# SEAME-pt/Team02-ObjectDetection

Hardware: NVIDIA B200
Metric: MobileNetV2UNet inference images/s (higher is better)
Workload: dtype bf16

## Files before the change

team02-objectdetection_b200/csrc/common.cuh:

```cuda
#pragma once
#include <cuda_runtime.h>
#include <cuda_bf16.h>
#include <cuda.h>
#include <stdint.h>
#include <stdio.h>

#include "../../include/b200seg.h"

namespace b200 {

int set_error(int code, const char* fmt, ...);
int check_launch(const char* what);
int sm_count();

int pdl_mode();
template <typename... KA, typename... A>
inline cudaError_t launch_pdl_if(bool on, void (*kern)(KA...), dim3 grid, dim3 block, size_t smem, cudaStream_t st, A... args) {
  cudaLaunchConfig_t cfg = {};
  cfg.gridDim = grid;
  cfg.blockDim = block;
  cfg.dynamicSmemBytes = smem;
  cfg.stream = st;
  cudaLaunchAttribute at[1];
  at[0].id = cudaLaunchAttributeProgrammaticStreamSerialization;
  at[0].val.programmaticStreamSerializationAllowed = 1;
  cfg.attrs = at;
  cfg.numAttrs = on ? 1 : 0;
  return cudaLaunchKernelEx(&cfg, kern, KA(args)...);
}
template <typename... KA, typename... A>
inline cudaError_t launch_pdl(void (*kern)(KA...), dim3 grid, dim3 block, size_t smem, cudaStream_t st, A... args) {
  const int m = pdl_mode();
  return launch_pdl_if(m == 1 || m == 3, kern, grid, block, smem, st, args...);
}

#define B200_REQUIRE(cond, ...)                                   \
  do {                                                            \
    if (!(cond)) return ::b200::set_error(-1, __VA_ARGS__);       \
  } while (0)

int make_tmap_bf16(CUtensorMap* out, const void* base, int rank, const uint64_t* dims,
                   const uint64_t* strides_bytes, const uint32_t* box, int swizzle128,
                   const uint32_t* elem_strides = nullptr);

#ifdef __CUDACC__

__device__ __forceinline__ uint32_t smem_u32(const void* p) {
  return static_cast<uint32_t>(__cvta_generic_to_shared(p));
}
__device__ __forceinline__ uint64_t globaltimer_ns() {
  uint64_t t;
  asm volatile("mov.u64 %0, %%globaltimer;" : "=l"(t));
  return t;
}

__device__ __forceinline__ void mbar_init(uint64_t* bar, uint32_t count) {
  asm volatile("mbarrier.init.shared::cta.b64 [%0], %1;" ::"r"(smem_u32(bar)), "r"(count) : "memory");
}
__device__ __forceinline__ void fence_barrier_init() {
  asm volatile("fence.mbarrier_init.release.cluster;" ::: "memory");
}
__device__ __forceinline__ void mbar_arrive_expect_tx(uint64_t* bar, uint32_t bytes) {
  asm volatile("mbarrier.arrive.expect_tx.shared::cta.b64 _, [%0], %1;" ::"r"(smem_u32(bar)), "r"(bytes)
               : "memory");
}
__device__ __forceinline__ void mbar_arrive(uint64_t* bar) {
  asm volatile("mbarrier.arrive.shared::cta.b64 _, [%0];" ::"r"(smem_u32(bar)) : "memory");
}
__device__ __forceinline__ bool mbar_try_wait(uint64_t* bar, uint32_t parity) {
  uint32_t ok;
  asm volatile(
      "{\n\t.reg .pred p;\n\t"
      "mbarrier.try_wait.parity.shared::cta.b64 p, [%1], %2;\n\t"
      "selp.u32 %0, 1, 0, p;\n\t}"
      : "=r"(ok)
      : "r"(smem_u32(bar)), "r"(parity)
      : "memory");
  return ok != 0;
}
__device__ __forceinline__ void mbar_wait(uint64_t* bar, uint32_t parity, int tag = 0) {
  if (mbar_try_wait(bar, parity)) return;
  const uint64_t t0 = globaltimer_ns();
  uint32_t spins = 0;
  while (!mbar_try_wait(bar, parity)) {
    if ((++spins & 0x3ff) == 0 && globaltimer_ns() - t0 > 2000000000ull) {
      printf("b200seg: mbarrier wait timeout tag=%d block=(%d,%d) thread=%d parity=%u\n", tag, blockIdx.x,
             blockIdx.y, threadIdx.x, parity);
      __trap();
    }
  }
}

__device__ __forceinline__ void pdl_wait() { asm volatile("griddepcontrol.wait;" ::: "memory"); }
__device__ __forceinline__ void pdl_trigger() { asm volatile("griddepcontrol.launch_dependents;" ::: "memory"); }

__device__ __forceinline__ bool elect_one() {
  uint32_t pred;
  asm volatile(
      "{\n\t.reg .pred P;\n\t"
      "elect.sync _|P, 0xffffffff;\n\t"
      "selp.u32 %0, 1, 0, P;\n\t}"
      : "=r"(pred));
  return pred != 0;
}

__device__ __forceinline__ void fence_proxy_async_smem() {
  asm volatile("fence.proxy.async.shared::cta;" ::: "memory");
}
__device__ __forceinline__ void tc_fence_before() { asm volatile("tcgen05.fence::before_thread_sync;" ::: "memory"); }
__device__ __forceinline__ void tc_fence_after() { asm volatile("tcgen05.fence::after_thread_sync;" ::: "memory"); }
__device__ __forceinline__ void named_bar_sync(int id, int nthreads) {
  asm volatile("bar.sync %0, %1;" ::"r"(id), "r"(nthreads) : "memory");
}

__device__ __forceinline__ void tma_prefetch_desc(const CUtensorMap* m) {
  asm volatile("prefetch.tensormap [%0];" ::"l"(m) : "memory");
}
__device__ __forceinline__ void tma_load_3d(void* dst, const CUtensorMap* m, uint64_t* bar, int c0, int c1,
                                            int c2) {
  asm volatile(
      "cp.async.bulk.tensor.3d.shared::cluster.global.mbarrier::complete_tx::bytes [%0], [%1, {%3, %4, %5}], [%2];"
      ::"r"(smem_u32(dst)), "l"(m), "r"(smem_u32(bar)), "r"(c0), "r"(c1), "r"(c2)
      : "memory");
}
__device__ __forceinline__ void tma_load_4d(void* dst, const CUtensorMap* m, uint64_t* bar, int c0, int c1,
                                            int c2, int c3) {
  asm volatile(
      "cp.async.bulk.tensor.4d.shared::cluster.global.mbarrier::complete_tx::bytes [%0], [%1, {%3, %4, %5, %6}], [%2];"
      ::"r"(smem_u32(dst)), "l"(m), "r"(smem_u32(bar)), "r"(c0), "r"(c1), "r"(c2), "r"(c3)
      : "memory");
}
__device__ __forceinline__ void tma_store_4d(const CUtensorMap* m, const void* src, int c0, int c1, int c2,
                                             int c3) {
  asm volatile("cp.async.bulk.tensor.4d.global.shared::cta.bulk_group [%0, {%2, %3, %4, %5}], [%1];" ::"l"(m),
               "r"(smem_u32(src)), "r"(c0), "r"(c1), "r"(c2), "r"(c3)
               : "memory");
}
__device__ __forceinline__ void tma_store_commit() { asm volatile("cp.async.bulk.commit_group;" ::: "memory"); }
__device__ __forceinline__ void tma_store_wait_all() { asm volatile("cp.async.bulk.wait_group 0;" ::: "memory"); }

__device__ __forceinline__ void tmem_alloc(uint32_t* dst_smem, uint32_t ncols) {
  asm volatile("tcgen05.alloc.cta_group::1.sync.aligned.shared::cta.b32 [%0], %1;" ::"r"(smem_u32(dst_smem)),
               "r"(ncols)
               : "memory");
}
__device__ __forceinline__ void tmem_relinquish() {
  asm volatile("tcgen05.relinquish_alloc_permit.cta_group::1.sync.aligned;" ::: "memory");
}
__device__ __forceinline__ void tmem_dealloc(uint32_t taddr, uint32_t ncols) {
  asm volatile("tcgen05.dealloc.cta_group::1.sync.aligned.b32 %0, %1;" ::"r"(taddr), "r"(ncols) : "memory");
}
__device__ __forceinline__ void umma_bf16(uint32_t d_tmem, uint64_t a_desc, uint64_t b_desc, uint32_t idesc,
                                          uint32_t accumulate) {
  asm volatile(
      "{\n\t.reg .pred p;\n\t"
      "setp.ne.b32 p, %4, 0;\n\t"
      "tcgen05.mma.cta_group::1.kind::f16 [%0], %1, %2, %3, p;\n\t}"
      ::"r"(d_tmem), "l"(a_desc), "l"(b_desc), "r"(idesc), "r"(accumulate)
      : "memory");
}
__device__ __forceinline__ void umma_bf16_lohi(uint32_t d_tmem, uint32_t a_lo, uint32_t b_lo, uint32_t desc_hi,
                                               uint32_t idesc, uint32_t accumulate) {
  asm volatile(
      "{\n\t.reg .pred p;\n\t.reg .b64 da, db;\n\t"
      "setp.ne.b32 p, %5, 0;\n\t"
      "mov.b64 da, {%1, %3};\n\t"
      "mov.b64 db, {%2, %3};\n\t"
      "tcgen05.mma.cta_group::1.kind::f16 [%0], da, db, %4, p;\n\t}"
      ::"r"(d_tmem), "r"(a_lo), "r"(b_lo), "r"(desc_hi), "r"(idesc), "r"(accumulate)
      : "memory");
}
__device__ __forceinline__ void umma_commit(uint64_t* bar) {
  asm volatile("tcgen05.commit.cta_group::1.mbarrier::arrive::one.shared::cluster.b64 [%0];" ::"r"(smem_u32(bar))
               : "memory");
}
__device__ __forceinline__ void tmem_ld16(uint32_t taddr, uint32_t (&r)[16]) {
  asm volatile(
      "tcgen05.ld.sync.aligned.32x32b.x16.b32 {%0, %1, %2, %3, %4, %5, %6, %7, %8, %9, %10, %11, %12, %13, %14, %15}, [%16];"
      : "=r"(r[0]), "=r"(r[1]), "=r"(r[2]), "=r"(r[3]), "=r"(r[4]), "=r"(r[5]), "=r"(r[6]), "=r"(r[7]),
        "=r"(r[8]), "=r"(r[9]), "=r"(r[10]), "=r"(r[11]), "=r"(r[12]), "=r"(r[13]), "=r"(r[14]), "=r"(r[15])
      : "r"(taddr)
      : "memory");
}
__device__ __forceinline__ void tmem_ld8(uint32_t taddr, uint32_t (&r)[16]) {
  asm volatile("tcgen05.ld.sync.aligned.32x32b.x8.b32 {%0, %1, %2, %3, %4, %5, %6, %7}, [%8];"
               : "=r"(r[0]), "=r"(r[1]), "=r"(r[2]), "=r"(r[3]), "=r"(r[4]), "=r"(r[5]), "=r"(r[6]), "=r"(r[7])
               : "r"(taddr)
               : "memory");
}
__device__ __forceinline__ void tmem_ld_wait() { asm volatile("tcgen05.wait::ld.sync.aligned;" ::: "memory"); }

__device__ __forceinline__ uint64_t umma_desc_k128(uint32_t smem_addr) {
  uint64_t d = 0;
  d |= (uint64_t)((smem_addr & 0x3FFFF) >> 4);
  d |= (uint64_t)1 << 16;
  d |= (uint64_t)(1024 >> 4) << 32;
  d |= (uint64_t)1 << 46;
  d |= (uint64_t)2 << 61;
  return d;
}
__device__ __forceinline__ uint64_t umma_desc_nosw(uint32_t smem_addr, uint32_t lbo_bytes, uint32_t sbo_bytes) {
  uint64_t d = 0;
  d |= (uint64_t)((smem_addr & 0x3FFFF) >> 4);
  d |= (uint64_t)(lbo_bytes >> 4) << 16;
  d |= (uint64_t)(sbo_bytes >> 4) << 32;
  d |= (uint64_t)1 << 46;
  return d;
}
__host__ __device__ __forceinline__ uint32_t umma_idesc_bf16(int M, int N) {
  return (1u << 4) | (1u << 7) | (1u << 10) | ((uint32_t)(N >> 3) << 17) | ((uint32_t)(M >> 4) << 24);
}

template <int ACT>
__device__ __forceinline__ float apply_act(float v) {
  if (ACT == B200SEG_ACT_RELU) return fmaxf(v, 0.f);
  if (ACT == B200SEG_ACT_RELU6) return fminf(fmaxf(v, 0.f), 6.f);
  return v;
}
__device__ __forceinline__ float apply_act_rt(float v, int act) {
  if (act == B200SEG_ACT_RELU) return fmaxf(v, 0.f);
  if (act == B200SEG_ACT_RELU6) return fminf(fmaxf(v, 0.f), 6.f);
  return v;
}
__device__ __forceinline__ uint32_t pack_bf16x2(float lo, float hi) {
  __nv_bfloat162 h = __floats2bfloat162_rn(lo, hi);
  return *reinterpret_cast<uint32_t*>(&h);
}
__device__ __forceinline__ float bf16lo(uint32_t u) { return __uint_as_float(u << 16); }
__device__ __forceinline__ float bf16hi(uint32_t u) { return __uint_as_float(u & 0xffff0000u); }

__device__ __forceinline__ float fma_bf16_lo(uint32_t a, uint32_t b, float c) {
  float d;
  asm("{.reg .b16 al, ah, bl, bh; mov.b32 {al, ah}, %1; mov.b32 {bl, bh}, %2; fma.rn.f32.bf16 %0, al, bl, %3;}"
      : "=f"(d) : "r"(a), "r"(b), "f"(c));
  return d;
}
__device__ __forceinline__ float fma_bf16_hi(uint32_t a, uint32_t b, float c) {
  float d;
  asm("{.reg .b16 al, ah, bl, bh; mov.b32 {al, ah}, %1; mov.b32 {bl, bh}, %2; fma.rn.f32.bf16 %0, ah, bh, %3;}"
      : "=f"(d) : "r"(a), "r"(b), "f"(c));
  return d;
}

template <typename T>
struct Vec16;
template <>
struct Vec16<float> {
  static constexpr int N = 4;
  typedef float4 Raw;
  float v[4];
  static __device__ __forceinline__ Raw ldraw(const float* p) { return __ldg(reinterpret_cast<const float4*>(p)); }
  __device__ __forceinline__ void unpack(const Raw& t) { v[0] = t.x; v[1] = t.y; v[2] = t.z; v[3] = t.w; }
  __device__ __forceinline__ void unpack_dep(const Raw& t, uint32_t) { unpack(t); }
  __device__ __forceinline__ void load(const float* p) { unpack(ldraw(p)); }
  __device__ __forceinline__ void store(float* p) const {
    *reinterpret_cast<float4*>(p) = make_float4(v[0], v[1], v[2], v[3]);
  }
};
template <>
struct Vec16<__nv_bfloat16> {
  static constexpr int N = 8;
  typedef uint4 Raw;
  float v[8];
  static __device__ __forceinline__ Raw ldraw(const __nv_bfloat16* p) {
    uint4 t;
    asm volatile("ld.global.nc.v4.u32 {%0, %1, %2, %3}, [%4];" : "=r"(t.x), "=r"(t.y), "=r"(t.z), "=r"(t.w) : "l"(p));
    return t;
  }
  __device__ __forceinline__ void unpack(const Raw& t) {
    v[0] = bf16lo(t.x); v[1] = bf16hi(t.x); v[2] = bf16lo(t.y); v[3] = bf16hi(t.y);
    v[4] = bf16lo(t.z); v[5] = bf16hi(t.z); v[6] = bf16lo(t.w); v[7] = bf16hi(t.w);
  }
  __device__ __forceinline__ void unpack_dep(const Raw& t, uint32_t dep) {
    v[0] = __uint_as_float((t.x << 16) + dep); v[1] = __uint_as_float((t.x & 0xffff0000u) | dep);
    v[2] = __uint_as_float((t.y << 16) + dep); v[3] = __uint_as_float((t.y & 0xffff0000u) | dep);
    v[4] = __uint_as_float((t.z << 16) + dep); v[5] = __uint_as_float((t.z & 0xffff0000u) | dep);
    v[6] = __uint_as_float((t.w << 16) + dep); v[7] = __uint_as_float((t.w & 0xffff0000u) | dep);
  }
  __device__ __forceinline__ void load(const __nv_bfloat16* p) { unpack(ldraw(p)); }
  __device__ __forceinline__ void store(__nv_bfloat16* p) const {
    uint4 t;
    t.x = pack_bf16x2(v[0], v[1]); t.y = pack_bf16x2(v[2], v[3]);
    t.z = pack_bf16x2(v[4], v[5]); t.w = pack_bf16x2(v[6], v[7]);
    *reinterpret_cast<uint4*>(p) = t;
  }
};

template <typename T> __device__ __forceinline__ float to_f32(T v);
template <> __device__ __forceinline__ float to_f32<float>(float v) { return v; }
template <> __device__ __forceinline__ float to_f32<__nv_bfloat16>(__nv_bfloat16 v) { return __bfloat162float(v); }
template <typename T> __device__ __forceinline__ T from_f32(float v);
template <> __device__ __forceinline__ float from_f32<float>(float v) { return v; }
template <> __device__ __forceinline__ __nv_bfloat16 from_f32<__nv_bfloat16>(float v) { return __float2bfloat16_rn(v); }

#endif

}
```

team02-objectdetection_b200/csrc/conv_tc.cu:

```cuda
#include "common.cuh"

namespace b200 {

struct ConvTcArgs {
  const float* bias;
  const void* res;
  void* y;
  int taps, Cin, Cout;
  int W, H, B;
  int BW, BH;
  int tiles_w, tiles_h;
  int block_n, n_tiles;
  int k_chunks;
  int stages;
  int act;
  int tma_store;
  int tmem_cols;
  int halo;
  int b_resident;
  int pdl_early;
  int n_sbuf;
  int halo_bo;
  int dw;
  int stride;
  int a_stage_bytes, b_stage_bytes;
  int mpair;
  int acc_bufs;
  long long m_tiles;
  long long total_tiles;
};

constexpr int TC_THREADS = 192;
constexpr int TILE_BYTES = 128 * 128;
constexpr int HALO_BYTES = 17 * 1024;

__device__ __forceinline__ uint64_t umma_desc_k128_off(uint32_t smem_addr) {
  return umma_desc_k128(smem_addr) | ((uint64_t)((smem_addr >> 7) & 7u) << 49);
}

template <int MPAIR>
__global__ void __launch_bounds__(TC_THREADS, 1)
conv_tc_kernel(const __grid_constant__ CUtensorMap tmA, const __grid_constant__ CUtensorMap tmB,
               const __grid_constant__ CUtensorMap tmC, const ConvTcArgs a) {
  extern __shared__ uint8_t smem_raw[];
  uint8_t* smem = smem_raw + ((1024u - (smem_u32(smem_raw) & 1023u)) & 1023u);

  const int warp = threadIdx.x >> 5, lane = threadIdx.x & 31;
  const int n_boxes = (a.block_n + 63) >> 6;
  const int kb_per_tile = a.halo ? a.k_chunks * 3 : a.k_chunks * a.taps;
  const int b_tiles_resident = a.taps * a.k_chunks;
  const int b_tile_bytes = a.block_n * 128;

  uint8_t* sA = smem;
  const int a_stride = MPAIR * a.a_stage_bytes;
  uint8_t* sB = sA + a.stages * a_stride;
  uint8_t* sOut = sB + (a.b_resident ? b_tiles_resident * b_tile_bytes : a.stages * a.b_stage_bytes);
  float* sBias = reinterpret_cast<float*>(sOut + a.n_sbuf * n_boxes * TILE_BYTES);
  uint64_t* full = reinterpret_cast<uint64_t*>(sBias + 256);
  uint64_t* empty = full + 8;
  uint64_t* acc_full = empty + 8;
  uint64_t* acc_empty = acc_full + 2;
  uint64_t* b_full = acc_empty + 2;
  uint32_t* tmem_slot = reinterpret_cast<uint32_t*>(b_full + 1);

  if (a.pdl_early) pdl_trigger();
  if (warp == 0 && lane == 0) {
    tma_prefetch_desc(&tmA);
    tma_prefetch_desc(&tmB);
    if (a.tma_store) tma_prefetch_desc(&tmC);
    for (int i = 0; i < a.stages; ++i) {
      mbar_init(&full[i], 1);
      mbar_init(&empty[i], 1);
    }
    for (int i = 0; i < 2; ++i) {
      mbar_init(&acc_full[i], 1);
      mbar_init(&acc_empty[i], 128);
    }
    mbar_init(b_full, 1);
    fence_barrier_init();
  }
  if (warp == 1) {
    tmem_alloc(tmem_slot, (uint32_t)a.tmem_cols);
    tmem_relinquish();
  }
  tc_fence_before();
  __syncthreads();
  tc_fence_after();
  const uint32_t tmem_base = *tmem_slot;
  const int rows = a.BW * a.BH;

  if (warp == 0) {
    if (a.b_resident && lane == 0) {
      mbar_arrive_expect_tx(b_full, (uint32_t)(b_tiles_resident * b_tile_bytes));
      for (int t = 0; t < a.taps; ++t)
        for (int c = 0; c < a.k_chunks; ++c)
          tma_load_3d(sB + (t * a.k_chunks + c) * b_tile_bytes, &tmB, b_full, c * 64, t, 0);
    }
    pdl_wait();
    int s = 0;
    uint32_t ph = 0;
    const int n_outer = a.halo ? a.k_chunks : a.taps;
    const int n_inner = a.halo ? 3 : a.k_chunks;
    const uint32_t tx_bytes = a.halo ? (uint32_t)MPAIR * 130u * 128u + (a.b_resident ? 0u : 3u * (uint32_t)b_tile_bytes)
                                     : (uint32_t)(MPAIR * rows * 128 + (a.b_resident ? 0 : b_tile_bytes));
    for (long long tile = blockIdx.x; tile < a.total_tiles; tile += gridDim.x) {
      const int n_tile = (int)(tile % a.n_tiles);
      const int n0 = n_tile * a.block_n;
      int w0v[MPAIR], h0v[MPAIR], bbv[MPAIR];
#pragma unroll
      for (int j = 0; j < MPAIR; ++j) {
        long long mt = (tile / a.n_tiles) * MPAIR + j;
        w0v[j] = (int)(mt % a.tiles_w) * a.BW; mt /= a.tiles_w;
        h0v[j] = (int)(mt % a.tiles_h) * a.BH;
        bbv[j] = (int)(mt / a.tiles_h);
      }
      for (int o = 0; o < n_outer; ++o) {
        for (int i = 0; i < n_inner; ++i) {
          mbar_wait(&empty[s], ph ^ 1u, 1);
          if (lane == 0) {
            mbar_arrive_expect_tx(&full[s], tx_bytes);
            if (a.halo) {
              const int chunk = o, dh = i;
              const int ach = a.dw ? n_tile : chunk;
#pragma unroll
              for (int j = 0; j < MPAIR; ++j)
                tma_load_4d(sA + s * a_stride + j * a.a_stage_bytes, &tmA, &full[s], ach * 64, w0v[j] - 1,
                            h0v[j] + dh - 1, bbv[j]);
              if (!a.b_resident)
                for (int dw = 0; dw < 3; ++dw)
                  tma_load_3d(sB + s * a.b_stage_bytes + dw * b_tile_bytes, &tmB, &full[s], a.dw ? 0 : chunk * 64,
                              dh * 3 + dw, n0);
            } else {
              const int tap = o, chunk = i;
              const int ach = a.dw ? n_tile : chunk;
              int dw = 0, dh = 0;
              if (a.taps == 9) { dh = tap / 3 - 1; dw = tap - (dh + 1) * 3 - 1; }
#pragma unroll
              for (int j = 0; j < MPAIR; ++j)
                tma_load_4d(sA + s * a_stride + j * a.a_stage_bytes, &tmA, &full[s], ach * 64, w0v[j] * a.stride + dw,
                            h0v[j] * a.stride + dh, bbv[j]);
              if (!a.b_resident)
                tma_load_3d(sB + s * a.b_stage_bytes, &tmB, &full[s], a.dw ? 0 : chunk * 64, tap, n0);
            }
          }
          __syncwarp();
          if (++s == a.stages) { s = 0; ph ^= 1u; }
        }
      }
    }
  } else if (warp == 1) {
    const uint32_t idesc = umma_idesc_bf16(128, a.block_n);
    const uint32_t desc_hi = (uint32_t)(umma_desc_k128(0) >> 32);
    const uint32_t a_lo0 = (uint32_t)umma_desc_k128(smem_u32(sA));
    const uint32_t b_lo0 = (uint32_t)umma_desc_k128(smem_u32(sB));
    const uint32_t a_stage16 = (uint32_t)a_stride >> 4, a_tile16 = (uint32_t)a.a_stage_bytes >> 4;
    const uint32_t b_stage16 = (uint32_t)a.b_stage_bytes >> 4;
    const uint32_t b_tile16 = (uint32_t)b_tile_bytes >> 4;
    const int n_outer = a.halo ? a.k_chunks : a.taps;
    const int n_inner = a.halo ? 3 : a.k_chunks;
    if (a.b_resident) mbar_wait(b_full, 0, 5);
    int s = 0;
    uint32_t ph = 0;
    int it = 0;
    for (long long tile = blockIdx.x; tile < a.total_tiles; tile += gridDim.x, ++it) {
      const int ab = a.acc_bufs == 2 ? (it & 1) : 0;
      const uint32_t aph = (uint32_t)(a.acc_bufs == 2 ? (it >> 1) : it) & 1u;
      mbar_wait(&acc_empty[ab], aph ^ 1u, 6);
      tc_fence_after();
      const uint32_t tacc0 = tmem_base + (uint32_t)(ab * MPAIR * a.block_n);
      const int n_tile = a.dw ? (int)(tile % a.n_tiles) : 0;
      uint32_t first = 0;
      for (int o = 0; o < n_outer; ++o) {
        for (int i = 0; i < n_inner; ++i) {
          const int chunk = a.halo ? o : i;
          const int ksteps = (min(64, a.Cin - (a.dw ? n_tile : chunk) * 64) + 15) >> 4;
          const uint32_t a_lo = a_lo0 + (uint32_t)s * a_stage16;
          mbar_wait(&full[s], ph, 2);
          tc_fence_after();
          if (elect_one()) {
            if (a.halo) {
              const int dh = i;
#pragma unroll
              for (int j = 0; j < MPAIR; ++j) {
                const uint32_t tacc = tacc0 + (uint32_t)(j * a.block_n);
                uint32_t fj = first;
#pragma unroll
                for (int dw = 0; dw < 3; ++dw) {
                  const int tap = dh * 3 + dw;
                  const uint32_t al = a_lo + (uint32_t)j * a_tile16 + (uint32_t)dw * 8u;
                  const uint32_t bl = a.b_resident ? b_lo0 + (uint32_t)(tap * a.k_chunks + chunk) * b_tile16
                                                   : b_lo0 + (uint32_t)s * b_stage16 + (uint32_t)dw * b_tile16;
#pragma unroll
                  for (int k = 0; k < 4; ++k)
                    if (k < ksteps) { umma_bf16_lohi(tacc, al + 2u * k, bl + 2u * k, desc_hi, idesc, fj); fj = 1u; }
                }
              }
            } else {
              const int tap = o;
              const uint32_t bl = a.b_resident ? b_lo0 + (uint32_t)(tap * a.k_chunks + chunk) * b_tile16
                                               : b_lo0 + (uint32_t)s * b_stage16;
#pragma unroll
              for (int j = 0; j < MPAIR; ++j) {
                const uint32_t tacc = tacc0 + (uint32_t)(j * a.block_n);
                const uint32_t al = a_lo + (uint32_t)j * a_tile16;
                uint32_t fj = first;
#pragma unroll
                for (int k = 0; k < 4; ++k)
                  if (k < ksteps) { umma_bf16_lohi(tacc, al + 2u * k, bl + 2u * k, desc_hi, idesc, fj); fj = 1u; }
              }
            }
            first = 1u;
            umma_commit(&empty[s]);
            if (o == n_outer - 1 && i == n_inner - 1) umma_commit(&acc_full[ab]);
          }
          __syncwarp();
          if (++s == a.stages) { s = 0; ph ^= 1u; }
        }
      }
    }
  } else {
    const int et = threadIdx.x - 64;
    const int q = warp & 3;
    const int r = q * 32 + lane;
    const int hl = r / a.BW, wl = r - hl * a.BW;
    const float act_lo = (a.act != B200SEG_ACT_NONE) ? 0.f : -INFINITY;
    const float act_hi = (a.act == B200SEG_ACT_RELU6) ? 6.f : INFINITY;
    const bool vec32 = (a.Cout & 15) == 0;
    pdl_wait();
    int it = 0;
    int cur_n_tile = -1;
    for (long long tile = blockIdx.x; tile < a.total_tiles; tile += gridDim.x, ++it) {
      const int n_tile = (int)(tile % a.n_tiles);
      const int n0 = n_tile * a.block_n;
      const int ab = a.acc_bufs == 2 ? (it & 1) : 0;
      const uint32_t aph = (uint32_t)(a.acc_bufs == 2 ? (it >> 1) : it) & 1u;
      int w0 = 0, h0 = 0, bb = 0;
      uint8_t* stg = sOut + (a.n_sbuf > 1 ? (it % a.n_sbuf) : 0) * n_boxes * TILE_BYTES;

      if (n_tile != cur_n_tile) {
        named_bar_sync(2, 128);
        for (int i = et; i < a.block_n; i += 128) sBias[i] = (a.bias && n0 + i < a.Cout) ? a.bias[n0 + i] : 0.f;
        cur_n_tile = n_tile;
        named_bar_sync(2, 128);
      }
      mbar_wait(&acc_full[ab], aph, 3);
      tc_fence_after();

      for (int j = 0; j < MPAIR; ++j) {
      {
        long long mt = (tile / a.n_tiles) * MPAIR + j;
        w0 = (int)(mt % a.tiles_w) * a.BW; mt /= a.tiles_w;
        h0 = (int)(mt % a.tiles_h) * a.BH;
        bb = (int)(mt / a.tiles_h);
      }
      const bool row_ok = r < rows && (h0 + hl) < a.H && (w0 + wl) < a.W && bb < a.B;
      const long long pix = ((long long)bb * a.H + (h0 + hl)) * a.W + (w0 + wl);
      const uint32_t trow = tmem_base + ((uint32_t)(q * 32) << 16) + (uint32_t)((ab * MPAIR + j) * a.block_n);
      const __nv_bfloat16* rp = reinterpret_cast<const __nv_bfloat16*>(a.res) + pix * a.Cout + n0;
      __nv_bfloat16* yp = reinterpret_cast<__nv_bfloat16*>(a.y) + pix * a.Cout + n0;

      auto process = [&](const uint32_t (&vv)[16], const int c0) {
        float f[16];
#pragma unroll
        for (int i = 0; i < 16; i += 4) {
          const float4 b4 = *reinterpret_cast<const float4*>(sBias + c0 + i);
          f[i] = fminf(fmaxf(__uint_as_float(vv[i]) + b4.x, act_lo), act_hi);
          f[i + 1] = fminf(fmaxf(__uint_as_float(vv[i + 1]) + b4.y, act_lo), act_hi);
          f[i + 2] = fminf(fmaxf(__uint_as_float(vv[i + 2]) + b4.z, act_lo), act_hi);
          f[i + 3] = fminf(fmaxf(__uint_as_float(vv[i + 3]) + b4.w, act_lo), act_hi);
        }
        const bool c_ok0 = n0 + c0 < a.Cout, c_ok1 = n0 + c0 + 8 < a.Cout;
        if (a.res != nullptr && row_ok && c_ok0) {
          uint32_t t[8];
          if (vec32) {
            asm volatile("ld.global.nc.v8.b32 {%0,%1,%2,%3,%4,%5,%6,%7}, [%8];"
                         : "=r"(t[0]), "=r"(t[1]), "=r"(t[2]), "=r"(t[3]), "=r"(t[4]), "=r"(t[5]), "=r"(t[6]), "=r"(t[7])
                         : "l"(rp + c0));
          } else {
            const uint4 u0 = __ldg(reinterpret_cast<const uint4*>(rp + c0));
            uint4 u1 = make_uint4(0, 0, 0, 0);
            if (c_ok1) u1 = __ldg(reinterpret_cast<const uint4*>(rp + c0 + 8));
            t[0] = u0.x; t[1] = u0.y; t[2] = u0.z; t[3] = u0.w; t[4] = u1.x; t[5] = u1.y; t[6] = u1.z; t[7] = u1.w;
          }
#pragma unroll
          for (int i = 0; i < 8; ++i) { f[2 * i] += bf16lo(t[i]); f[2 * i + 1] += bf16hi(t[i]); }
        }
        uint32_t o[8];
#pragma unroll
        for (int i = 0; i < 8; ++i) o[i] = pack_bf16x2(f[2 * i], f[2 * i + 1]);
        if (a.tma_store) {
          const int bx = c0 >> 6, j = (c0 & 63) >> 3;
          uint8_t* rowp = stg + bx * TILE_BYTES + r * 128;
          *reinterpret_cast<uint4*>(rowp + ((j ^ (r & 7)) << 4)) = make_uint4(o[0], o[1], o[2], o[3]);
          *reinterpret_cast<uint4*>(rowp + (((j + 1) ^ (r & 7)) << 4)) = make_uint4(o[4], o[5], o[6], o[7]);
        } else if (row_ok && c_ok0) {
          if (vec32) {
            asm volatile("st.global.v8.b32 [%0], {%1,%2,%3,%4,%5,%6,%7,%8};" ::"l"(yp + c0), "r"(o[0]), "r"(o[1]),
                         "r"(o[2]), "r"(o[3]), "r"(o[4]), "r"(o[5]), "r"(o[6]), "r"(o[7])
                         : "memory");
          } else {
            *reinterpret_cast<uint4*>(yp + c0) = make_uint4(o[0], o[1], o[2], o[3]);
            if (c_ok1) *reinterpret_cast<uint4*>(yp + c0 + 8) = make_uint4(o[4], o[5], o[6], o[7]);
          }
        }
      };
      uint32_t va[16], vb[16];
      tmem_ld16(trow, va);
      const int nch = a.block_n >> 4;
      for (int ch = 0; ch < nch; ch += 2) {
        tmem_ld_wait();
        if (ch + 1 < nch) tmem_ld16(trow + (uint32_t)((ch + 1) << 4), vb);
        process(va, ch << 4);
        if (ch + 1 < nch) {
          tmem_ld_wait();
          if (ch + 2 < nch) tmem_ld16(trow + (uint32_t)((ch + 2) << 4), va);
          process(vb, (ch + 1) << 4);
        }
      }
      }
      tc_fence_before();
      mbar_arrive(&acc_empty[ab]);
      if (a.tma_store) {
        fence_proxy_async_smem();
        if (et == 0) {
          if (a.n_sbuf >= 4) asm volatile("cp.async.bulk.wait_group.read 2;" ::: "memory");
          else if (a.n_sbuf == 3) asm volatile("cp.async.bulk.wait_group.read 1;" ::: "memory");
          else if (a.n_sbuf == 2) asm volatile("cp.async.bulk.wait_group.read 0;" ::: "memory");
        }
        named_bar_sync(1, 128);
        if (et == 0) {
          for (int bx = 0; bx < n_boxes; ++bx)
            if (n0 + bx * 64 < a.Cout) tma_store_4d(&tmC, stg + bx * TILE_BYTES, n0 + bx * 64, w0, h0, bb);
          tma_store_commit();
          if (a.n_sbuf == 1) asm volatile("cp.async.bulk.wait_group.read 0;" ::: "memory");
        }
        if (a.n_sbuf == 1) named_bar_sync(1, 128);
      }
    }
    if (a.tma_store && et == 0) tma_store_wait_all();
    tc_fence_before();
  }
  if (!a.pdl_early) pdl_trigger();
  __syncthreads();
  if (warp == 1) {
    tc_fence_after();
    tmem_dealloc(tmem_base, (uint32_t)a.tmem_cols);
  }
}

static void pick_tile(int W, int H, int* BW, int* BH) {
  double best = -1.0;
  int bw_best = 1, bh_best = 1;
  const int wmax = W < 128 ? W : 128;
  for (int bw = wmax; bw >= 1; --bw) {
    int bh = 128 / bw;
    if (bh > H) bh = H;
    if (bh < 1) bh = 1;
    const long long tiles = (long long)((W + bw - 1) / bw) * ((H + bh - 1) / bh);
    const double eff = (double)W * H / ((double)tiles * 128.0);
    if (eff > best + 1e-9) { best = eff; bw_best = bw; bh_best = bh; }
    if (bw <= 8 && best > 0) break;
  }
  *BW = bw_best; *BH = bh_best;
}

}

using namespace b200;

static int launch_conv_tc(const void* x, const void* w, const float* bias, const void* res, void* y, int B, int H,
                          int W, int Cin, int Cout, int taps, int stride, int dwmode, int act, int flags,
                          cudaStream_t stream) {
  const int Ho = (H - 1) / stride + 1, Wo = (W - 1) / stride + 1;
  ConvTcArgs a;
  a.bias = bias; a.res = res; a.y = y;
  a.taps = taps; a.Cin = Cin; a.Cout = Cout;
  a.dw = dwmode; a.stride = stride;
  a.halo = (taps == 9 && stride == 1 && W >= 96 && !(flags & 2)) ? 1 : 0;
  if (taps == 1) {
    const long long M = (long long)B * H * W;
    B200_REQUIRE(M < (1ll << 31), "conv_tc: too many pixels");
    a.W = (int)M; a.H = 1; a.B = 1;
  } else {
    a.W = Wo; a.H = Ho; a.B = B;
  }
  if (a.halo) { a.BW = Wo < 128 ? Wo : 128; a.BH = 1; }
  else pick_tile(a.W, a.H, &a.BW, &a.BH);
  a.tiles_w = (a.W + a.BW - 1) / a.BW;
  a.tiles_h = (a.H + a.BH - 1) / a.BH;
  if (dwmode) {
    a.block_n = Cout >= 64 ? 64 : ((Cout + 15) & ~15);
    a.n_tiles = (Cout + 63) / 64;
    a.k_chunks = 1;
  } else {
    if (Cout <= 256) {
      a.block_n = (Cout + 15) & ~15; a.n_tiles = 1;
    } else {
      int nt = (Cout + 255) / 256;
      int bn = (((Cout + nt - 1) / nt) + 63) & ~63;
      a.block_n = bn; a.n_tiles = (Cout + bn - 1) / bn;
    }
    a.k_chunks = (Cin + 63) / 64;
  }
  a.act = act;
  a.tma_store = flags & 1;
  a.halo_bo = (flags & 16) ? 1 : 0;
  a.tmem_cols = 32;
  while (a.tmem_cols < 2 * a.block_n) a.tmem_cols <<= 1;

  const int n_boxes = (a.block_n + 63) / 64;
  const int b_tile = a.block_n * 128;
  const int smem_cap = 227 * 1024 - 1024  - 1024  - 256 ;
  a.a_stage_bytes = a.halo ? HALO_BYTES : TILE_BYTES;
  const int kb_per_tile = a.halo ? a.k_chunks * 3 : a.k_chunks * taps;
  const int b_all = taps * a.k_chunks * b_tile;
  a.n_sbuf = 0;
  if (a.tma_store) {
    a.n_sbuf = (flags & 8) ? 1 : 3;
    while (a.n_sbuf > 1 && a.n_sbuf * n_boxes * TILE_BYTES > 64 * 1024) --a.n_sbuf;
  }
  const int out_bytes = a.n_sbuf * n_boxes * TILE_BYTES;
  a.b_resident = (a.n_tiles == 1 && !(flags & 4) && b_all <= 80 * 1024 && b_all + out_bytes + 2 * a.a_stage_bytes <= smem_cap) ? 1 : 0;
  a.b_stage_bytes = a.b_resident ? 0 : (a.halo ? 3 * b_tile : b_tile);
  a.m_tiles = (long long)a.tiles_w * a.tiles_h * a.B;
  a.mpair = (!a.b_resident && taps * a.k_chunks >= 27 && !a.tma_store && !(flags & 32) && a.m_tiles >= 2) ? 2 : 1;
  a.acc_bufs = (a.mpair == 1 || a.block_n <= 64) ? 2 : 1;
  a.tmem_cols = 32;
  while (a.tmem_cols < a.acc_bufs * a.mpair * a.block_n) a.tmem_cols <<= 1;
  const int per_stage = a.mpair * a.a_stage_bytes + a.b_stage_bytes;
  const int fixed = out_bytes + (a.b_resident ? b_all : 0);
  int want = kb_per_tile <= 3 ? 4 : 6;
  if ((flags >> 16) & 0xf) want = (flags >> 16) & 0xf;
  int stages = (smem_cap - fixed) / per_stage;
  if (stages > want) stages = want;
  if (stages > 8) stages = 8;
  if (!((flags >> 16) & 0xf) && 2 * a.tmem_cols <= 512) {
    const int half_cap = (227 * 1024) / 2 - 1024 - (1024 + 1024 + 256);
    int st2 = (half_cap - fixed) / per_stage;
    if (st2 > want) st2 = want;
    if (st2 >= 2) stages = st2;
  }
  B200_REQUIRE(stages >= 1, "conv_tc: tile does not fit in shared memory (Cin=%d Cout=%d taps=%d)", Cin, Cout, taps);
  a.stages = stages;
  const int smem = fixed + stages * per_stage + 1024 + 1024 + 256;
  B200_REQUIRE(smem <= 227 * 1024, "conv_tc: smem %d too large", smem);
  a.total_tiles = ((a.m_tiles + a.mpair - 1) / a.mpair) * a.n_tiles;

  CUtensorMap tmA, tmB, tmC;
  {
    const uint64_t iw = taps == 1 ? (uint64_t)a.W : (uint64_t)W, ih = taps == 1 ? 1 : (uint64_t)H, ib = taps == 1 ? 1 : (uint64_t)B;
    uint64_t dims[4] = {(uint64_t)Cin, iw, ih, ib};
    uint64_t str[3] = {(uint64_t)Cin * 2, (uint64_t)Cin * 2 * iw, (uint64_t)Cin * 2 * iw * ih};
    uint32_t box[4] = {64, (uint32_t)(a.halo ? 130 : a.BW * stride), (uint32_t)(a.BH * stride), 1};
    uint32_t es[4] = {1, (uint32_t)stride, (uint32_t)stride, 1};
    int rc = make_tmap_bf16(&tmA, x, 4, dims, str, box, 1, es);
    if (rc) return rc;
  }
  {
    uint64_t dims[3] = {(uint64_t)(dwmode ? 64 : Cin), (uint64_t)taps, (uint64_t)Cout};
    uint64_t str[2] = {dims[0] * 2, dims[0] * 2 * taps};
    uint32_t box[3] = {64, 1, (uint32_t)a.block_n};
    int rc = make_tmap_bf16(&tmB, w, 3, dims, str, box, 1, nullptr);
    if (rc) return rc;
  }
  {
    uint64_t dims[4] = {(uint64_t)Cout, (uint64_t)a.W, (uint64_t)a.H, (uint64_t)a.B};
    uint64_t str[3] = {(uint64_t)Cout * 2, (uint64_t)Cout * 2 * a.W, (uint64_t)Cout * 2 * a.W * a.H};
    uint32_t box[4] = {64, (uint32_t)a.BW, (uint32_t)a.BH, 1};
    int rc = make_tmap_bf16(&tmC, y, 4, dims, str, box, 1, nullptr);
    if (rc) return rc;
  }
  int dev = 0;
  cudaGetDevice(&dev);
  static bool attr_set[64] = {false};
  if (dev >= 0 && dev < 64 && !attr_set[dev]) {
    cudaError_t e = cudaFuncSetAttribute(conv_tc_kernel<1>, cudaFuncAttributeMaxDynamicSharedMemorySize, 227 * 1024);
    if (e == cudaSuccess) e = cudaFuncSetAttribute(conv_tc_kernel<2>, cudaFuncAttributeMaxDynamicSharedMemorySize, 227 * 1024);
    if (e != cudaSuccess) return set_error((int)e, "conv_tc: cudaFuncSetAttribute: %s", cudaGetErrorString(e));
    attr_set[dev] = true;
  }
  int per_sm = (227 * 1024) / (smem + 1024);
  if (per_sm > 512 / a.tmem_cols) per_sm = 512 / a.tmem_cols;
  if (per_sm > 2) per_sm = 2;
  if ((flags >> 20) & 0x3) per_sm = (flags >> 20) & 0x3;
  if (per_sm < 1) per_sm = 1;
  long long grid = (long long)sm_count() * per_sm;
  if ((flags >> 8) & 0xff) grid = (long long)((flags >> 8) & 0xff) * 4;
  if (grid > a.total_tiles) grid = a.total_tiles;
  a.pdl_early = pdl_mode() != 3;
  if (a.mpair == 2) launch_pdl_if(pdl_mode() > 0, conv_tc_kernel<2>, dim3((unsigned)grid), dim3(TC_THREADS), (size_t)smem, stream, tmA, tmB, tmC, a);
  else launch_pdl_if(pdl_mode() > 0, conv_tc_kernel<1>, dim3((unsigned)grid), dim3(TC_THREADS), (size_t)smem, stream, tmA, tmB, tmC, a);
  return check_launch("conv_tc");
}

extern "C" int b200seg_conv_tc(const void* x, const void* w, const float* bias, const void* res, void* y, int B,
                               int H, int W, int Cin, int Cout, int taps, int act, int flags,
                               b200seg_stream_t s) {
  B200_REQUIRE(taps == 1 || taps == 9, "conv_tc: taps=%d (1 or 9)", taps);
  B200_REQUIRE(Cin > 0 && Cin % 8 == 0, "conv_tc: Cin=%d must be a positive multiple of 8", Cin);
  B200_REQUIRE(Cout > 0 && Cout % 8 == 0, "conv_tc: Cout=%d must be a positive multiple of 8", Cout);
  B200_REQUIRE(B > 0 && H > 0 && W > 0, "conv_tc: empty tensor");
  B200_REQUIRE(x && w && y, "conv_tc: null pointer");
  return launch_conv_tc(x, w, bias, res, y, B, H, W, Cin, Cout, taps, 1, 0, act, flags, (cudaStream_t)s);
}

extern "C" int b200seg_dwconv3x3_tc(const void* x, const void* wdiag, const float* bias, void* y, int B, int H,
                                    int W, int C, int stride, int act, int flags, b200seg_stream_t s) {
  B200_REQUIRE(C > 0 && C % 8 == 0, "dwconv3x3_tc: C=%d must be a positive multiple of 8", C);
  B200_REQUIRE(stride == 1 || stride == 2, "dwconv3x3_tc: stride=%d", stride);
  B200_REQUIRE(B > 0 && H > 0 && W > 0, "dwconv3x3_tc: empty tensor");
  B200_REQUIRE(x && wdiag && y, "dwconv3x3_tc: null pointer");
  return launch_conv_tc(x, wdiag, bias, nullptr, y, B, H, W, C, C, 9, stride, 1, act, flags, (cudaStream_t)s);
}
```

Measured before the change: 34550.

## Add CTA-pair (cta_group::2) UMMA path for dense 3x3 convs

Adds a 2-CTA cluster variant of the tcgen05 conv kernel. Each CTA loads half of the weight N-tile and its own M tile, and the leader CTA issues 256-row pair MMAs with multicast commits. The variant is selected automatically for dense 3x3 stride-1 convs with one N tile and at least two K chunks. The intent is to halve per-CTA weight smem traffic and use larger MMAs. In exchange it adds cluster synchronisation, cross-CTA barrier arrivals and halves the number of independent work units, which can hurt load balance on small layers.

```diff
diff --git a/team02-objectdetection_b200/csrc/common.cuh b/team02-objectdetection_b200/csrc/common.cuh
--- a/team02-objectdetection_b200/csrc/common.cuh
+++ b/team02-objectdetection_b200/csrc/common.cuh
@@ -174,6 +174,65 @@
   asm volatile("tcgen05.commit.cta_group::1.mbarrier::arrive::one.shared::cluster.b64 [%0];" ::"r"(smem_u32(bar))
                : "memory");
 }
+__device__ __forceinline__ uint32_t cluster_ctarank() {
+  uint32_t r;
+  asm volatile("mov.u32 %0, %%cluster_ctarank;" : "=r"(r));
+  return r;
+}
+__device__ __forceinline__ void cluster_sync() {
+  asm volatile("barrier.cluster.arrive.release.aligned;\n\tbarrier.cluster.wait.acquire.aligned;" ::: "memory");
+}
+__device__ __forceinline__ uint32_t mapa_shared(uint32_t smem_addr, uint32_t rank) {
+  uint32_t r;
+  asm volatile("mapa.shared::cluster.u32 %0, %1, %2;" : "=r"(r) : "r"(smem_addr), "r"(rank));
+  return r;
+}
+__device__ __forceinline__ void mbar_arrive_cluster(uint32_t cluster_addr) {
+  asm volatile("mbarrier.arrive.release.cluster.shared::cluster.b64 _, [%0];" ::"r"(cluster_addr) : "memory");
+}
+__device__ __forceinline__ void tma_load_3d_pair(void* dst, const CUtensorMap* m, uint32_t bar_cluster, int c0, int c1,
+                                                 int c2) {
+  asm volatile(
+      "cp.async.bulk.tensor.3d.cta_group::2.shared::cluster.global.mbarrier::complete_tx::bytes [%0], [%1, {%3, %4, %5}], [%2];"
+      ::"r"(smem_u32(dst)), "l"(m), "r"(bar_cluster), "r"(c0), "r"(c1), "r"(c2)
+      : "memory");
+}
+__device__ __forceinline__ void tma_load_4d_pair(void* dst, const CUtensorMap* m, uint32_t bar_cluster, int c0, int c1,
+                                                 int c2, int c3) {
+  asm volatile(
+      "cp.async.bulk.tensor.4d.cta_group::2.shared::cluster.global.mbarrier::complete_tx::bytes [%0], [%1, {%3, %4, %5, %6}], [%2];"
+      ::"r"(smem_u32(dst)), "l"(m), "r"(bar_cluster), "r"(c0), "r"(c1), "r"(c2), "r"(c3)
+      : "memory");
+}
+__device__ __forceinline__ void tmem_alloc_pair(uint32_t* dst_smem, uint32_t ncols) {
+  asm volatile("tcgen05.alloc.cta_group::2.sync.aligned.shared::cta.b32 [%0], %1;" ::"r"(smem_u32(dst_smem)),
+               "r"(ncols)
+               : "memory");
+}
+__device__ __forceinline__ void tmem_relinquish_pair() {
+  asm volatile("tcgen05.relinquish_alloc_permit.cta_group::2.sync.aligned;" ::: "memory");
+}
+__device__ __forceinline__ void tmem_dealloc_pair(uint32_t taddr, uint32_t ncols) {
+  asm volatile("tcgen05.dealloc.cta_group::2.sync.aligned.b32 %0, %1;" ::"r"(taddr), "r"(ncols) : "memory");
+}
+__device__ __forceinline__ void umma_bf16_lohi_pair(uint32_t d_tmem, uint32_t a_lo, uint32_t b_lo, uint32_t desc_hi,
+                                                    uint32_t idesc, uint32_t accumulate) {
+  asm volatile(
+      "{\n\t.reg .pred p;\n\t.reg .b64 da, db;\n\t"
+      "setp.ne.b32 p, %5, 0;\n\t"
+      "mov.b64 da, {%1, %3};\n\t"
+      "mov.b64 db, {%2, %3};\n\t"
+      "tcgen05.mma.cta_group::2.kind::f16 [%0], da, db, %4, p;\n\t}"
+      ::"r"(d_tmem), "r"(a_lo), "r"(b_lo), "r"(desc_hi), "r"(idesc), "r"(accumulate)
+      : "memory");
+}
+__device__ __forceinline__ void umma_commit_pair(uint64_t* bar) {
+  asm volatile(
+      "tcgen05.commit.cta_group::2.mbarrier::arrive::one.shared::cluster.multicast::cluster.b64 [%0], %1;"
+      ::"r"(smem_u32(bar)), "h"((uint16_t)3)
+      : "memory");
+}
+
 __device__ __forceinline__ void tmem_ld16(uint32_t taddr, uint32_t (&r)[16]) {
   asm volatile(
       "tcgen05.ld.sync.aligned.32x32b.x16.b32 {%0, %1, %2, %3, %4, %5, %6, %7, %8, %9, %10, %11, %12, %13, %14, %15}, [%16];"
diff --git a/team02-objectdetection_b200/csrc/conv_tc.cu b/team02-objectdetection_b200/csrc/conv_tc.cu
--- a/team02-objectdetection_b200/csrc/conv_tc.cu
+++ b/team02-objectdetection_b200/csrc/conv_tc.cu
@@ -38,7 +38,7 @@
   return umma_desc_k128(smem_addr) | ((uint64_t)((smem_addr >> 7) & 7u) << 49);
 }
 
-template <int MPAIR>
+template <int MPAIR, int CG>
 __global__ void __launch_bounds__(TC_THREADS, 1)
 conv_tc_kernel(const __grid_constant__ CUtensorMap tmA, const __grid_constant__ CUtensorMap tmB,
                const __grid_constant__ CUtensorMap tmC, const ConvTcArgs a) {
@@ -49,7 +49,8 @@
   const int n_boxes = (a.block_n + 63) >> 6;
   const int kb_per_tile = a.halo ? a.k_chunks * 3 : a.k_chunks * a.taps;
   const int b_tiles_resident = a.taps * a.k_chunks;
-  const int b_tile_bytes = a.block_n * 128;
+  const int b_tile_bytes = a.block_n / CG * 128;
+  const uint32_t rank = CG == 2 ? cluster_ctarank() : 0u;
 
   uint8_t* sA = smem;
   const int a_stride = MPAIR * a.a_stage_bytes;
@@ -74,27 +75,42 @@
     }
     for (int i = 0; i < 2; ++i) {
       mbar_init(&acc_full[i], 1);
-      mbar_init(&acc_empty[i], 128);
+      mbar_init(&acc_empty[i], 128 * CG);
     }
     mbar_init(b_full, 1);
     fence_barrier_init();
   }
   if (warp == 1) {
-    tmem_alloc(tmem_slot, (uint32_t)a.tmem_cols);
-    tmem_relinquish();
+    if constexpr (CG == 2) {
+      tmem_alloc_pair(tmem_slot, (uint32_t)a.tmem_cols);
+      tmem_relinquish_pair();
+    } else {
+      tmem_alloc(tmem_slot, (uint32_t)a.tmem_cols);
+      tmem_relinquish();
+    }
   }
   tc_fence_before();
   __syncthreads();
+  if constexpr (CG == 2) cluster_sync();
   tc_fence_after();
   const uint32_t tmem_base = *tmem_slot;
   const int rows = a.BW * a.BH;
 
   if (warp == 0) {
+    auto load_b = [&](void* dst, uint64_t* bar, int c0, int c1, int c2) {
+      if constexpr (CG == 2) tma_load_3d_pair(dst, &tmB, mapa_shared(smem_u32(bar), 0), c0, c1, c2);
+      else tma_load_3d(dst, &tmB, bar, c0, c1, c2);
+    };
+    auto load_a = [&](void* dst, uint64_t* bar, int c0, int c1, int c2, int c3) {
+      if constexpr (CG == 2) tma_load_4d_pair(dst, &tmA, mapa_shared(smem_u32(bar), 0), c0, c1, c2, c3);
+      else tma_load_4d(dst, &tmA, bar, c0, c1, c2, c3);
+    };
+    const int n_half = (int)rank * (a.block_n / CG);
     if (a.b_resident && lane == 0) {
-      mbar_arrive_expect_tx(b_full, (uint32_t)(b_tiles_resident * b_tile_bytes));
+      if (rank == 0) mbar_arrive_expect_tx(b_full, (uint32_t)(CG * b_tiles_resident * b_tile_bytes));
       for (int t = 0; t < a.taps; ++t)
         for (int c = 0; c < a.k_chunks; ++c)
-          tma_load_3d(sB + (t * a.k_chunks + c) * b_tile_bytes, &tmB, b_full, c * 64, t, 0);
+          load_b(sB + (t * a.k_chunks + c) * b_tile_bytes, b_full, c * 64, t, n_half);
     }
     pdl_wait();
     int s = 0;
@@ -103,13 +119,13 @@
     const int n_inner = a.halo ? 3 : a.k_chunks;
     const uint32_t tx_bytes = a.halo ? (uint32_t)MPAIR * 130u * 128u + (a.b_resident ? 0u : 3u * (uint32_t)b_tile_bytes)
                                      : (uint32_t)(MPAIR * rows * 128 + (a.b_resident ? 0 : b_tile_bytes));
-    for (long long tile = blockIdx.x; tile < a.total_tiles; tile += gridDim.x) {
+    for (long long tile = blockIdx.x / CG; tile < a.total_tiles; tile += gridDim.x / CG) {
       const int n_tile = (int)(tile % a.n_tiles);
-      const int n0 = n_tile * a.block_n;
+      const int n0 = n_tile * a.block_n + n_half;
       int w0v[MPAIR], h0v[MPAIR], bbv[MPAIR];
 #pragma unroll
       for (int j = 0; j < MPAIR; ++j) {
-        long long mt = (tile / a.n_tiles) * MPAIR + j;
+        long long mt = ((tile / a.n_tiles) * CG + rank) * MPAIR + j;
         w0v[j] = (int)(mt % a.tiles_w) * a.BW; mt /= a.tiles_w;
         h0v[j] = (int)(mt % a.tiles_h) * a.BH;
         bbv[j] = (int)(mt / a.tiles_h);
@@ -118,18 +134,18 @@
         for (int i = 0; i < n_inner; ++i) {
           mbar_wait(&empty[s], ph ^ 1u, 1);
           if (lane == 0) {
-            mbar_arrive_expect_tx(&full[s], tx_bytes);
+            if (rank == 0) mbar_arrive_expect_tx(&full[s], CG * tx_bytes);
             if (a.halo) {
               const int chunk = o, dh = i;
               const int ach = a.dw ? n_tile : chunk;
 #pragma unroll
               for (int j = 0; j < MPAIR; ++j)
-                tma_load_4d(sA + s * a_stride + j * a.a_stage_bytes, &tmA, &full[s], ach * 64, w0v[j] - 1,
-                            h0v[j] + dh - 1, bbv[j]);
+                load_a(sA + s * a_stride + j * a.a_stage_bytes, &full[s], ach * 64, w0v[j] - 1, h0v[j] + dh - 1,
+                       bbv[j]);
               if (!a.b_resident)
                 for (int dw = 0; dw < 3; ++dw)
-                  tma_load_3d(sB + s * a.b_stage_bytes + dw * b_tile_bytes, &tmB, &full[s], a.dw ? 0 : chunk * 64,
-                              dh * 3 + dw, n0);
+                  load_b(sB + s * a.b_stage_bytes + dw * b_tile_bytes, &full[s], a.dw ? 0 : chunk * 64, dh * 3 + dw,
+                         n0);
             } else {
               const int tap = o, chunk = i;
               const int ach = a.dw ? n_tile : chunk;
@@ -137,10 +153,10 @@
               if (a.taps == 9) { dh = tap / 3 - 1; dw = tap - (dh + 1) * 3 - 1; }
 #pragma unroll
               for (int j = 0; j < MPAIR; ++j)
-                tma_load_4d(sA + s * a_stride + j * a.a_stage_bytes, &tmA, &full[s], ach * 64, w0v[j] * a.stride + dw,
-                            h0v[j] * a.stride + dh, bbv[j]);
+                load_a(sA + s * a_stride + j * a.a_stage_bytes, &full[s], ach * 64, w0v[j] * a.stride + dw,
+                       h0v[j] * a.stride + dh, bbv[j]);
               if (!a.b_resident)
-                tma_load_3d(sB + s * a.b_stage_bytes, &tmB, &full[s], a.dw ? 0 : chunk * 64, tap, n0);
+                load_b(sB + s * a.b_stage_bytes, &full[s], a.dw ? 0 : chunk * 64, tap, n0);
             }
           }
           __syncwarp();
@@ -148,9 +164,17 @@
         }
       }
     }
-  } else if (warp == 1) {
-    const uint32_t idesc = umma_idesc_bf16(128, a.block_n);
+  } else if (warp == 1 && rank == 0) {
+    const uint32_t idesc = umma_idesc_bf16(128 * CG, a.block_n);
     const uint32_t desc_hi = (uint32_t)(umma_desc_k128(0) >> 32);
+    auto mma = [&](uint32_t tacc, uint32_t al, uint32_t bl, uint32_t acc) {
+      if constexpr (CG == 2) umma_bf16_lohi_pair(tacc, al, bl, desc_hi, idesc, acc);
+      else umma_bf16_lohi(tacc, al, bl, desc_hi, idesc, acc);
+    };
+    auto commit = [&](uint64_t* bar) {
+      if constexpr (CG == 2) umma_commit_pair(bar);
+      else umma_commit(bar);
+    };
     const uint32_t a_lo0 = (uint32_t)umma_desc_k128(smem_u32(sA));
     const uint32_t b_lo0 = (uint32_t)umma_desc_k128(smem_u32(sB));
     const uint32_t a_stage16 = (uint32_t)a_stride >> 4, a_tile16 = (uint32_t)a.a_stage_bytes >> 4;
@@ -162,7 +186,7 @@
     int s = 0;
     uint32_t ph = 0;
     int it = 0;
-    for (long long tile = blockIdx.x; tile < a.total_tiles; tile += gridDim.x, ++it) {
+    for (long long tile = blockIdx.x / CG; tile < a.total_tiles; tile += gridDim.x / CG, ++it) {
       const int ab = a.acc_bufs == 2 ? (it & 1) : 0;
       const uint32_t aph = (uint32_t)(a.acc_bufs == 2 ? (it >> 1) : it) & 1u;
       mbar_wait(&acc_empty[ab], aph ^ 1u, 6);
@@ -192,7 +216,7 @@
                                                    : b_lo0 + (uint32_t)s * b_stage16 + (uint32_t)dw * b_tile16;
 #pragma unroll
                   for (int k = 0; k < 4; ++k)
-                    if (k < ksteps) { umma_bf16_lohi(tacc, al + 2u * k, bl + 2u * k, desc_hi, idesc, fj); fj = 1u; }
+                    if (k < ksteps) { mma(tacc, al + 2u * k, bl + 2u * k, fj); fj = 1u; }
                 }
               }
             } else {
@@ -206,19 +230,19 @@
                 uint32_t fj = first;
 #pragma unroll
                 for (int k = 0; k < 4; ++k)
-                  if (k < ksteps) { umma_bf16_lohi(tacc, al + 2u * k, bl + 2u * k, desc_hi, idesc, fj); fj = 1u; }
+                  if (k < ksteps) { mma(tacc, al + 2u * k, bl + 2u * k, fj); fj = 1u; }
               }
             }
             first = 1u;
-            umma_commit(&empty[s]);
-            if (o == n_outer - 1 && i == n_inner - 1) umma_commit(&acc_full[ab]);
+            commit(&empty[s]);
+            if (o == n_outer - 1 && i == n_inner - 1) commit(&acc_full[ab]);
           }
           __syncwarp();
           if (++s == a.stages) { s = 0; ph ^= 1u; }
         }
       }
     }
-  } else {
+  } else if (CG == 1 || warp != 1) {
     const int et = threadIdx.x - 64;
     const int q = warp & 3;
     const int r = q * 32 + lane;
@@ -229,7 +253,7 @@
     pdl_wait();
     int it = 0;
     int cur_n_tile = -1;
-    for (long long tile = blockIdx.x; tile < a.total_tiles; tile += gridDim.x, ++it) {
+    for (long long tile = blockIdx.x / CG; tile < a.total_tiles; tile += gridDim.x / CG, ++it) {
       const int n_tile = (int)(tile % a.n_tiles);
       const int n0 = n_tile * a.block_n;
       const int ab = a.acc_bufs == 2 ? (it & 1) : 0;
@@ -248,7 +272,7 @@
 
       for (int j = 0; j < MPAIR; ++j) {
       {
-        long long mt = (tile / a.n_tiles) * MPAIR + j;
+        long long mt = ((tile / a.n_tiles) * CG + rank) * MPAIR + j;
         w0 = (int)(mt % a.tiles_w) * a.BW; mt /= a.tiles_w;
         h0 = (int)(mt % a.tiles_h) * a.BH;
         bb = (int)(mt / a.tiles_h);
@@ -319,7 +343,8 @@
       }
       }
       tc_fence_before();
-      mbar_arrive(&acc_empty[ab]);
+      if constexpr (CG == 2) mbar_arrive_cluster(mapa_shared(smem_u32(&acc_empty[ab]), 0));
+      else mbar_arrive(&acc_empty[ab]);
       if (a.tma_store) {
         fence_proxy_async_smem();
         if (et == 0) {
@@ -342,9 +367,11 @@
   }
   if (!a.pdl_early) pdl_trigger();
   __syncthreads();
+  if constexpr (CG == 2) cluster_sync();
   if (warp == 1) {
     tc_fence_after();
-    tmem_dealloc(tmem_base, (uint32_t)a.tmem_cols);
+    if constexpr (CG == 2) tmem_dealloc_pair(tmem_base, (uint32_t)a.tmem_cols);
+    else tmem_dealloc(tmem_base, (uint32_t)a.tmem_cols);
   }
 }
 
@@ -408,8 +435,16 @@
   a.tmem_cols = 32;
   while (a.tmem_cols < 2 * a.block_n) a.tmem_cols <<= 1;
 
+  const bool pair_ok = taps == 9 && !dwmode && stride == 1 && !a.tma_store && a.block_n % 32 == 0;
+  B200_REQUIRE(!((flags & 64) && (flags & 128)), "conv_tc: flags forbid and force the CTA-pair kernel");
+  B200_REQUIRE(!(flags & 128) || pair_ok,
+               "conv_tc: the CTA-pair kernel needs a dense 3x3 stride-1 conv, an N tile that is a multiple of 32 and "
+               "direct stores (Cout=%d block_n=%d flags=0x%x)", Cout, a.block_n, flags);
+  const bool pair_auto = a.k_chunks >= 2 && a.n_tiles == 1;
+  const int cg = (pair_ok && !(flags & 64) && ((flags & 128) || pair_auto)) ? 2 : 1;
+
   const int n_boxes = (a.block_n + 63) / 64;
-  const int b_tile = a.block_n * 128;
+  const int b_tile = a.block_n / cg * 128;
   const int smem_cap = 227 * 1024 - 1024  - 1024  - 256 ;
   a.a_stage_bytes = a.halo ? HALO_BYTES : TILE_BYTES;
   const int kb_per_tile = a.halo ? a.k_chunks * 3 : a.k_chunks * taps;
@@ -423,7 +458,7 @@
   a.b_resident = (a.n_tiles == 1 && !(flags & 4) && b_all <= 80 * 1024 && b_all + out_bytes + 2 * a.a_stage_bytes <= smem_cap) ? 1 : 0;
   a.b_stage_bytes = a.b_resident ? 0 : (a.halo ? 3 * b_tile : b_tile);
   a.m_tiles = (long long)a.tiles_w * a.tiles_h * a.B;
-  a.mpair = (!a.b_resident && taps * a.k_chunks >= 27 && !a.tma_store && !(flags & 32) && a.m_tiles >= 2) ? 2 : 1;
+  a.mpair = (!a.b_resident && taps * a.k_chunks >= 27 && !a.tma_store && !(flags & 32) && a.m_tiles >= 2 * cg) ? 2 : 1;
   a.acc_bufs = (a.mpair == 1 || a.block_n <= 64) ? 2 : 1;
   a.tmem_cols = 32;
   while (a.tmem_cols < a.acc_bufs * a.mpair * a.block_n) a.tmem_cols <<= 1;
@@ -444,7 +479,7 @@
   a.stages = stages;
   const int smem = fixed + stages * per_stage + 1024 + 1024 + 256;
   B200_REQUIRE(smem <= 227 * 1024, "conv_tc: smem %d too large", smem);
-  a.total_tiles = ((a.m_tiles + a.mpair - 1) / a.mpair) * a.n_tiles;
+  a.total_tiles = ((a.m_tiles + a.mpair * cg - 1) / (a.mpair * cg)) * a.n_tiles;
 
   CUtensorMap tmA, tmB, tmC;
   {
@@ -459,7 +494,7 @@
   {
     uint64_t dims[3] = {(uint64_t)(dwmode ? 64 : Cin), (uint64_t)taps, (uint64_t)Cout};
     uint64_t str[2] = {dims[0] * 2, dims[0] * 2 * taps};
-    uint32_t box[3] = {64, 1, (uint32_t)a.block_n};
+    uint32_t box[3] = {64, 1, (uint32_t)(a.block_n / cg)};
     int rc = make_tmap_bf16(&tmB, w, 3, dims, str, box, 1, nullptr);
     if (rc) return rc;
   }
@@ -474,8 +509,10 @@
   cudaGetDevice(&dev);
   static bool attr_set[64] = {false};
   if (dev >= 0 && dev < 64 && !attr_set[dev]) {
-    cudaError_t e = cudaFuncSetAttribute(conv_tc_kernel<1>, cudaFuncAttributeMaxDynamicSharedMemorySize, 227 * 1024);
-    if (e == cudaSuccess) e = cudaFuncSetAttribute(conv_tc_kernel<2>, cudaFuncAttributeMaxDynamicSharedMemorySize, 227 * 1024);
+    cudaError_t e = cudaFuncSetAttribute(conv_tc_kernel<1, 1>, cudaFuncAttributeMaxDynamicSharedMemorySize, 227 * 1024);
+    if (e == cudaSuccess) e = cudaFuncSetAttribute(conv_tc_kernel<2, 1>, cudaFuncAttributeMaxDynamicSharedMemorySize, 227 * 1024);
+    if (e == cudaSuccess) e = cudaFuncSetAttribute(conv_tc_kernel<1, 2>, cudaFuncAttributeMaxDynamicSharedMemorySize, 227 * 1024);
+    if (e == cudaSuccess) e = cudaFuncSetAttribute(conv_tc_kernel<2, 2>, cudaFuncAttributeMaxDynamicSharedMemorySize, 227 * 1024);
     if (e != cudaSuccess) return set_error((int)e, "conv_tc: cudaFuncSetAttribute: %s", cudaGetErrorString(e));
     attr_set[dev] = true;
   }
@@ -486,10 +523,29 @@
   if (per_sm < 1) per_sm = 1;
   long long grid = (long long)sm_count() * per_sm;
   if ((flags >> 8) & 0xff) grid = (long long)((flags >> 8) & 0xff) * 4;
+  a.pdl_early = pdl_mode() != 3;
+  if (cg == 2) {
+    grid /= 2;
+    if (grid > a.total_tiles) grid = a.total_tiles;
+    cudaLaunchConfig_t cfg = {};
+    cfg.gridDim = dim3((unsigned)(2 * grid));
+    cfg.blockDim = dim3(TC_THREADS);
+    cfg.dynamicSmemBytes = (size_t)smem;
+    cfg.stream = stream;
+    cudaLaunchAttribute at[2];
+    at[0].id = cudaLaunchAttributeClusterDimension;
+    at[0].val.clusterDim.x = 2; at[0].val.clusterDim.y = 1; at[0].val.clusterDim.z = 1;
+    at[1].id = cudaLaunchAttributeProgrammaticStreamSerialization;
+    at[1].val.programmaticStreamSerializationAllowed = 1;
+    cfg.attrs = at;
+    cfg.numAttrs = pdl_mode() > 0 ? 2 : 1;
+    if (a.mpair == 2) cudaLaunchKernelEx(&cfg, conv_tc_kernel<2, 2>, tmA, tmB, tmC, a);
+    else cudaLaunchKernelEx(&cfg, conv_tc_kernel<1, 2>, tmA, tmB, tmC, a);
+    return check_launch("conv_tc (CTA pairs)");
+  }
   if (grid > a.total_tiles) grid = a.total_tiles;
-  a.pdl_early = pdl_mode() != 3;
-  if (a.mpair == 2) launch_pdl_if(pdl_mode() > 0, conv_tc_kernel<2>, dim3((unsigned)grid), dim3(TC_THREADS), (size_t)smem, stream, tmA, tmB, tmC, a);
-  else launch_pdl_if(pdl_mode() > 0, conv_tc_kernel<1>, dim3((unsigned)grid), dim3(TC_THREADS), (size_t)smem, stream, tmA, tmB, tmC, a);
+  if (a.mpair == 2) launch_pdl_if(pdl_mode() > 0, conv_tc_kernel<2, 1>, dim3((unsigned)grid), dim3(TC_THREADS), (size_t)smem, stream, tmA, tmB, tmC, a);
+  else launch_pdl_if(pdl_mode() > 0, conv_tc_kernel<1, 1>, dim3((unsigned)grid), dim3(TC_THREADS), (size_t)smem, stream, tmA, tmB, tmC, a);
   return check_launch("conv_tc");
 }
 
```

Measured after the change: 35260 (median of 6 runs). 2.0% higher.
